# bytedance/particle-sfm

Measured on AMD Instinct MI355X. Metric: trajectory-points/s, higher is better.
Workload: dtype f32 sampling + f64 positions; 1 GPU; configs[1]: synthetic 100x(1920x1080) flow pairs, sample_ratio=2, flow_check + chaining + occlusion + id assignment, 1 sequence per GPU; frames=101, height=1080, width=1920, trajectories=2073277, parallelism=sequence-per-gpu x1, world_size=1

## Files before the change

### particle-sfm_amd/csrc/psfm_api.hip

```cpp
#include <stdarg.h>
#include <stdio.h>
#include <string.h>
#include <mutex>
#include <shared_mutex>
#include <atomic>
#include <chrono>
#include <stdlib.h>

#include "psfm_internal.h"

static thread_local char g_err[512] = "";
static std::shared_mutex g_dev_gate[16];
std::shared_mutex& psfm_device_gate(int device) { return g_dev_gate[device & 15]; }
static std::atomic<int> g_dev_waiters[16];
int psfm_gate_waiters(int device) { return g_dev_waiters[device & 15].load(std::memory_order_relaxed); }
void psfm_gate_waiters_add(int device, int d) { g_dev_waiters[device & 15].fetch_add(d, std::memory_order_relaxed); }
static int psfm_wants_persist(psfm_ctx* c, bool optimize, int h, int w, int ratio, bool fused)
{
    if (c->chain_mode == 1 || ratio < 1 || !psfm_frame_ok(h, w)) return 0;
    if (optimize) return c->resident_budget > 0 ? 0 : 1;
    const int64_t G = (int64_t)((w + ratio - 1) / ratio) * ((h + ratio - 1) / ratio);
    const int64_t P = (int64_t)h * w;
    const int maxb = psfm_persist_max_blocks(c);
    if (maxb <= 0 || (G + 255) / 256 > maxb) return 0;
// ... 81 lines not shown
void PsfmProfiler::reset()
{
    for (int k = 0; k < PSFM_PROF_KINDS; ++k) { total_ms[k] = 0; launches[k] = 0; }
}
void PsfmProfiler::destroy()
{
    collect();
    for (auto e : pool) (void)hipEventDestroy(e);
    pool.clear();
}

#define PSFM_CHECK_CTX(c)                                                     \
    do {                                                                      \
        if (!(c)) { psfm_set_error("ctx is NULL"); return PSFM_ERR_ARG; }     \
        PSFM_HIP(hipSetDevice((c)->device));                                  \
    } while (0)

extern "C" psfm_status psfm_ctx_create(int device, psfm_ctx** out)
{
    if (!out) { psfm_set_error("psfm_ctx_create: out is NULL"); return PSFM_ERR_ARG; }
    *out = nullptr;
    int n = 0;
    hipError_t e = hipGetDeviceCount(&n);
    if (e != hipSuccess || n <= 0) {
        (void)hipGetLastError();
        psfm_set_error("no HIP device available (%s); libpsfm_hip has no CPU fallback",
                       e != hipSuccess ? hipGetErrorString(e) : "device count 0");
        return PSFM_ERR_HIP;
    }
    if (device < 0 || device >= n) { psfm_set_error("device %d out of range [0,%d)", device, n); return PSFM_ERR_ARG; }
    PSFM_HIP(hipSetDevice(device));
    psfm_ctx* c = new psfm_ctx();
    c->device = device;
    c->host_pinned_bytes = 512 + sizeof(PsfmShard) * PSFM_NSHARD + 4096;
    e = hipHostMalloc(&c->host_pinned, c->host_pinned_bytes, hipHostMallocDefault);
    if (e != hipSuccess) { delete c; psfm_set_error("hipHostMalloc failed: %s", hipGetErrorString(e)); return PSFM_ERR_HIP; }
    *out = c;
    return PSFM_OK;
}

extern "C" psfm_status psfm_ctx_destroy(psfm_ctx* c)
{
    if (!c) return PSFM_OK;
    (void)hipSetDevice(c->device);
    PsfmBuf* bufs[] = {&c->log, &c->birth_frame, &c->birth_idx, &c->free_stack, &c->fin_keys, &c->fin_lanes,
                       &c->occupied, &c->counters, &c->shards, &c->survivors, &c->sort_keys, &c->sort_lanes, &c->sort_tmp,
                       &c->scan_tmp, &c->fin_marks, &c->res_birth, &c->res_len, &c->res_off, &c->res_xy, &c->sol_x, &c->sol_state,
                       &c->sol_partials, &c->sol_ctrl, &c->sol_misc, &c->sol_stats, &c->sol_fused, &c->sol_bar, &c->sol_list, &c->occ_own, &c->occ2_own,
                       &c->handoff, &c->seg_info, &c->seg_table, &c->persist_bar, &c->batch_tab, &c->batch_ws, &c->batch_fc, &c->win_ws, &c->flt_ids, &c->flt_birth, &c->flt_len, &c->flt_off, &c->flt_xy,
                       &c->mt_kp_off, &c->mt_q, &c->mt_pts, &c->mt_kp_ind, &c->mt_kp_xy, &c->mt_moff, &c->mt_keys, &c->mt_rows, &c->mt_gid, &c->mt_pairs,
                       &c->lb_state, &c->lb_first, &c->lb_flag, &c->lb_ws, &c->lb_ids, &c->lb_off, &c->lb_frames, &c->lb_xy, &c->lb_labels, &c->gt_flag};
    for (auto b : bufs) b->release();
    for (void*& q : c->peer_opened) { if (q) (void)hipIpcCloseMemHandle(q); q = nullptr; }
    c->peer_area.release();
    psfm_shard_abandon(c);
    c->prof.destroy();
    if (c->side_stream) (void)hipStreamDestroy(c->side_stream);
    if (c->redo_stream) (void)hipStreamDestroy(c->redo_stream);
    if (c->copy_stream) (void)hipStreamDestroy(c->copy_stream);
    if (c->copy_stream2) (void)hipStreamDestroy(c->copy_stream2);
    for (void* p : c->ingest_slots) (void)hipHostFree(p);
    for (hipEvent_t e : c->ingest_events) (void)hipEventDestroy(e);
    if (c->host_pinned) (void)hipHostFree(c->host_pinned);
    if (c->host_seg) (void)hipHostFree(c->host_seg);
    if (c->host_batch) (void)hipHostFree(c->host_batch);
    if (c->host_batch2) (void)hipHostFree(c->host_batch2);
    delete c;
    return PSFM_OK;
}
// ... 246 lines not shown
    psfm_status st;
    if ((st = psfm_track_dims(c, n_flows, h, w, ratio, -1, d)) != PSFM_OK) return st;
    const int64_t P = (int64_t)h * w;
    if ((st = psfm_track_alloc(c, d)) != PSFM_OK) return st;

    c->solve_stats.clear();
    c->res_n_traj = c->res_n_points = 0;
    c->res_n_flows = n_flows;
    c->pc_persist_ok = device_is_ours || c->resident_budget > 0;
    c->pc_giveups = 0;

    if (!optimize && c->chain_mode != 1) {
        const int maxb = psfm_persist_max_blocks(c);
        const int64_t need_blocks = (d.G + 255) / 256;
        if (maxb > 0 && need_blocks <= maxb && device_is_ours) {
            PsfmTrackDims dp = d;
            int64_t nb = need_blocks <= 256 ? 2 * need_blocks + 4 : need_blocks + need_blocks / 4;
            dp.nblk = (int)(nb < maxb ? nb : maxb);
            if (fuse_flows_b) {
                const int64_t fc_blocks = (P + 1023) / 1024;
                const int64_t want = fc_blocks < maxb ? fc_blocks : maxb;
                if (want > dp.nblk) dp.nblk = (int)want;
            }
            dp.cap = (int64_t)dp.nblk * (256 + psfm_persist_guests());
            dp.nsh = dp.nblk < PSFM_NSHARD ? dp.nblk : PSFM_NSHARD;
            dp.free_cap = (int)(((dp.nblk + dp.nsh - 1) / dp.nsh) * 256) + 1024;
            dp.seg_cap = (int)(d.traj_cap / dp.nblk) + 64;
            dp.spill_cap = (int)(d.traj_cap / 8) + 4096;
            const int64_t fin_total = (int64_t)dp.nblk * dp.seg_cap + dp.spill_cap;
            if ((st = c->log.ensure(sizeof(double2) * (size_t)(n_flows + 1) * dp.cap)) != PSFM_OK) return st;
            if ((st = c->free_stack.ensure(sizeof(int) * (size_t)dp.free_cap * PSFM_NSHARD * 2)) != PSFM_OK) return st;
            if ((st = c->fin_keys.ensure(sizeof(unsigned long long) * fin_total)) != PSFM_OK) return st;
            if ((st = c->fin_lanes.ensure(sizeof(int) * fin_total)) != PSFM_OK) return st;
            if ((st = c->handoff.ensure((size_t)dp.nblk * 256 * 24)) != PSFM_OK) return st;
            if ((st = c->seg_info.ensure(sizeof(int) * 2 * (size_t)dp.nblk)) != PSFM_OK) return st;
            if ((st = c->persist_bar.ensure((size_t)(4 * PSFM_NSHARD + 1) * 128)) != PSFM_OK) return st;
            if (pipe && (st = pipe->need(n_flows - 1, false, s)) != PSFM_OK) return st;
            bool fallback = false;
            {
                const bool trace = getenv("PSFM_TRACE") != nullptr;
                const auto t1 = std::chrono::steady_clock::now();
                st = psfm_launch_chain_persist(c, dp, flows, occ, occ_pitch, fuse_flows_b, fuse_thres, s);
                if (st == PSFM_ERR_CAPACITY) {
                    fallback = true;
                    st = PSFM_OK;
                } else {
                    if (st != PSFM_OK) return st;
                    c->prof.begin(PSFM_PROF_FINALIZE, s);
                    st = psfm_finalize_persist(c, dp, &fallback, s);
                    c->prof.end(s);
                }
                if (trace) {
                    const auto t2 = std::chrono::steady_clock::now();
                    fprintf(stderr, "[psfm %p] persistent loop: launch+finalize %.2f ms, fallback %d, overflow %d\n", (void*)c,
                            std::chrono::duration<double, std::milli>(t2 - t1).count(), (int)fallback,
                            ((PsfmCounters*)c->host_pinned)->overflow);
                }
            }
            if (st != PSFM_OK) return st;
            if (!fallback) {
                PSFM_HIP(hipStreamSynchronize(s));
                c->prof.collect();
                if (info) {
                    memset(info, 0, sizeof(*info));
                    info->n_traj = c->res_n_traj;
                    info->n_points = c->res_n_points;
                    info->n_lanes_peak = ((PsfmCounters*)c->host_pinned)->n_lanes;
                    info->lane_capacity = dp.cap;
                    info->chain_mode = 2;
                }
                return PSFM_OK;
            }
            c->prof.collect();
        }
    }
    if (fuse_flows_b) {
        c->prof.begin(PSFM_PROF_FLOW_CHECK, s);
        for (int f = 0; f < n_flows; ++f)
            if ((st = psfm_launch_flow_check(flows + (size_t)f * P * 2, fuse_flows_b + (size_t)f * P * 2, 1, h, w, fuse_thres,
                                             const_cast<uint8_t*>(occ) + (size_t)f * occ_pitch, nullptr, s)) != PSFM_OK) return st;
        c->prof.end(s);
    }
    if ((st = psfm_launch_track_init(c, d, s)) != PSFM_OK) return st;
    int64_t total_iters = 0;
    static const int check_env = getenv("PSFM_CHECK_FRAMES") ? atoi(getenv("PSFM_CHECK_FRAMES")) : 0;
    const int PSFM_CHECK = check_env >= 2 ? check_env : 16;
    std::vector<psfm_solve_stats> hstats((size_t)n_flows + 1);
    int first_unchecked = 1;
    if (optimize) {
// ... 308 lines not shown
```

### particle-sfm_amd/csrc/psfm_finalize.hip

```cpp
#include <cstring>
#include <stdio.h>
#include <rocprim/device/device_radix_sort.hpp>
#include <rocprim/device/device_scan.hpp>

#include "psfm_device.h"
#include "psfm_internal.h"

#define PSFM_BLOCK 256

__device__ __forceinline__ void psfm_collect_alive_body(
    const int* __restrict__ birth_frame, const int* __restrict__ birth_idx, PsfmCounters* __restrict__ ctr,
    PsfmShard* __restrict__ shards, unsigned long long* __restrict__ fin_keys, int* __restrict__ fin_lanes, int cap,
    int shard_cap, int last_time, int shift_b, int shift_d)
{
    __shared__ int s_cnt[PSFM_BLOCK / PSFM_WAVE];
    __shared__ int s_base;
    const int n_lanes = min(ctr->n_lanes, cap);
    if ((int)(blockIdx.x * PSFM_BLOCK) >= n_lanes) return;
    const int i = blockIdx.x * PSFM_BLOCK + threadIdx.x;
    int bf = -1;
    if (i < n_lanes) bf = birth_frame[i];
    const bool pending = bf <= -2;
    const bool alive = (bf >= 0) | pending;
    const int my_last = pending ? last_time - 1 : last_time;
// ... 380 lines not shown
#pragma unroll
            for (int k = 0; k < TILE_K; ++k) {
                const int t = k0 + k;
                if (t >= 1 && t < l) { pos.x = pos.x + (double)f[k].x; pos.y = pos.y + (double)f[k].y; }
                tile[tid][k] = pos;
            }
            s_pos[tid] = pos;
        }
        __syncthreads();
        const int kk = tid & (TILE_K - 1);
        for (int jj = tid / TILE_K; jj < TILE_J; jj += PSFM_BLOCK / TILE_K) {
            const int t = k0 + kk;
            if (t < s_len[jj]) out[s_off[jj] + t] = tile[jj][kk];
        }
        __syncthreads();
    }
}

static PsfmKeyFmt psfm_key_fmt(const PsfmTrackDims& d, unsigned* end_bit)
{
    PsfmKeyFmt f;
    f.shift_b = d.shift_b; f.shift_d = d.shift_d;
    const long long lmax = (long long)d.n_flows + 1;
    const long long tri_max = lmax * (lmax + 1) / 2 + lmax;
    int tri_bits = 1;
    while ((1ll << tri_bits) <= tri_max) ++tri_bits;
    f.use32 = (tri_bits + d.shift_b <= 32) ? 1 : 0;
    int tbits = 1;
    while ((1ll << tbits) < (long long)d.n_flows + 2) ++tbits;
    *end_bit = f.use32 ? (unsigned)(tri_bits + d.shift_b) : (unsigned)(d.shift_d + tbits);
    return f;
}

static bool psfm_own_sort(const PsfmKeyFmt& fmt, int64_t n)
{
    static const int on = getenv("PSFM_FIN_SORT") ? atoi(getenv("PSFM_FIN_SORT")) : 1;
    return on && fmt.use32 && n < (1ll << 31);
}
static bool psfm_records_in_first_half(const PsfmTrackDims& d, int64_t n)
{
    unsigned end_bit = 0;
    const PsfmKeyFmt fmt = psfm_key_fmt(d, &end_bit);
    return psfm_own_sort(fmt, n) && (psfm_sort_pairs32_passes(end_bit) % 2 == 0);
}

static psfm_status psfm_finalize_sorted(psfm_ctx* c, const PsfmTrackDims& d, int64_t n, int64_t npts, bool delta_log, hipStream_t s)
{
    psfm_status st;
    unsigned end_bit = 0;
    const PsfmKeyFmt fmt = psfm_key_fmt(d, &end_bit);
    int* l_in = c->sort_lanes.as<int>() + n;
    int* l_out = c->sort_lanes.as<int>();
    size_t tmp_bytes = 0, scan_bytes = 0;
    PSFM_HIP(rocprim::exclusive_scan(nullptr, scan_bytes, (int64_t*)nullptr, (int64_t*)nullptr, (int64_t)0,
                                     (size_t)(n + 1), rocprim::plus<int64_t>(), s));
    if (psfm_own_sort(fmt, n)) {
        if ((st = c->sort_tmp.ensure(scan_bytes)) != PSFM_OK) return st;
        if ((st = psfm_sort_pairs32(c, c->sort_keys.as<unsigned>(), l_out, c->sort_keys.as<unsigned>() + n, l_in, n, end_bit, s)) != PSFM_OK) return st;
    } else if (fmt.use32) {
        unsigned* k_in = c->sort_keys.as<unsigned>() + n;
        unsigned* k_out = c->sort_keys.as<unsigned>();
        PSFM_HIP(rocprim::radix_sort_pairs(nullptr, tmp_bytes, k_in, k_out, l_in, l_out, (size_t)n, 0u, end_bit, s));
        if ((st = c->sort_tmp.ensure(tmp_bytes > scan_bytes ? tmp_bytes : scan_bytes)) != PSFM_OK) return st;
        PSFM_HIP(rocprim::radix_sort_pairs(c->sort_tmp.p, tmp_bytes, k_in, k_out, l_in, l_out, (size_t)n, 0u, end_bit, s));
    } else {
        unsigned long long* k_in = c->sort_keys.as<unsigned long long>() + n;
        unsigned long long* k_out = c->sort_keys.as<unsigned long long>();
        PSFM_HIP(rocprim::radix_sort_pairs(nullptr, tmp_bytes, k_in, k_out, l_in, l_out, (size_t)n, 0u, end_bit, s));
        if ((st = c->sort_tmp.ensure(tmp_bytes > scan_bytes ? tmp_bytes : scan_bytes)) != PSFM_OK) return st;
        PSFM_HIP(rocprim::radix_sort_pairs(c->sort_tmp.p, tmp_bytes, k_in, k_out, l_in, l_out, (size_t)n, 0u, end_bit, s));
    }
    if ((st = c->res_birth.ensure(sizeof(int) * n)) != PSFM_OK) return st;
    if ((st = c->res_len.ensure(sizeof(int) * n)) != PSFM_OK) return st;
    if ((st = c->res_off.ensure(sizeof(int64_t) * (n + 1))) != PSFM_OK) return st;
    static const int plan_on = getenv("PSFM_FIN_PLAN") ? atoi(getenv("PSFM_FIN_PLAN")) : 1;
    const long long lmax = (long long)d.n_flows + 1;
    const long long ng = lmax * (lmax + 1) / 2 + lmax + 1;
    PsfmPlan pl;
    pl.gstart = nullptr; pl.goff = nullptr; pl.keys = (const void*)c->sort_keys.p; pl.use32 = fmt.use32; pl.shift_b = d.shift_b; pl.shift_d = d.shift_d;
    pl.birth_w = c->res_birth.as<int>(); pl.len_w = c->res_len.as<int>(); pl.off_w = c->res_off.as<int64_t>();
    if (plan_on && ng <= PSFM_PLAN_MAX_GROUPS && n < (1ll << 31)) {
        if ((st = c->scan_tmp.ensure((sizeof(int64_t) + sizeof(int)) * (size_t)ng)) != PSFM_OK) return st;
        int64_t* goff = c->scan_tmp.as<int64_t>();
        int* gstart = (int*)(goff + ng);
        const void* had = c->fin_marks.p;
        if ((st = c->fin_marks.ensure(sizeof(int) * (size_t)PSFM_PLAN_MAX_GROUPS)) != PSFM_OK) return st;
        if (!c->fin_marks_clean || had != c->fin_marks.p)
            PSFM_HIP(hipMemsetAsync(c->fin_marks.p, 0xff, sizeof(int) * (size_t)PSFM_PLAN_MAX_GROUPS, s));
        c->fin_marks_clean = false;
        hipLaunchKernelGGL(psfm_group_bounds_kernel, dim3((unsigned)((n + PSFM_BLOCK - 1) / PSFM_BLOCK)), dim3(PSFM_BLOCK), 0, s,
                           (const void*)c->sort_keys.p, n, fmt.use32, d.shift_b, d.shift_d, c->fin_marks.as<int>());
        hipLaunchKernelGGL(psfm_group_plan_kernel, dim3(1), dim3(PSFM_PLAN_BLOCK), 0, s, c->fin_marks.as<int>(), gstart, goff, (int)ng, n,
                           c->res_off.as<int64_t>() + n);
        PSFM_HIP(hipGetLastError());
        c->fin_marks_clean = true;
        pl.gstart = gstart; pl.goff = goff;
    } else {
        if ((st = c->scan_tmp.ensure(sizeof(int64_t) * (n + 1))) != PSFM_OK) return st;
        if (fmt.use32)
// ... 37 lines not shown
    PSFM_HIP(hipMemcpyAsync(hc, ctr, sizeof(PsfmCounters), hipMemcpyDeviceToHost, s));
    PSFM_HIP(hipMemcpyAsync(hs, shards, sizeof(PsfmShard) * PSFM_NSHARD, hipMemcpyDeviceToHost, s));
    PSFM_HIP(hipStreamSynchronize(s));
    PsfmShardOffsets so;
    int64_t n = 0, npts = 0;
    bool over = hc->overflow != 0;
    for (int k = 0; k < PSFM_NSHARD; ++k) npts += hs[k].points;
    for (int k = 0; k < PSFM_NSHARD; ++k) {
        if (hs[k].fin_cnt > d.shard_cap) over = true;
        so.count[k] = hs[k].fin_cnt > d.shard_cap ? d.shard_cap : hs[k].fin_cnt;
        so.start[k] = n;
        n += so.count[k];
    }
    if (over || hc->n_lanes > d.cap) {
        psfm_set_error("capacity exceeded: lanes used %d of %lld, trajectory records %lld of %lld (%d shards); "
                       "raise psfm_ctx_set_capacity", hc->n_lanes, (long long)d.cap, (long long)n,
                       (long long)d.traj_cap, PSFM_NSHARD);
        return PSFM_ERR_CAPACITY;
    }
    c->res_n_traj = n;
    c->res_n_points = 0;
    if (n == 0) return PSFM_OK;
    psfm_status st;
    if ((st = c->sort_keys.ensure(sizeof(unsigned long long) * n * 2)) != PSFM_OK) return st;
    if ((st = c->sort_lanes.ensure(sizeof(int) * n * 2)) != PSFM_OK) return st;
    unsigned end_bit_unused = 0;
    const PsfmKeyFmt fmt = psfm_key_fmt(d, &end_bit_unused);
    const int64_t half = psfm_records_in_first_half(d, n) ? 0 : n;
    unsigned long long* kdst = fmt.use32 ? (unsigned long long*)(c->sort_keys.as<unsigned>() + half) : c->sort_keys.as<unsigned long long>() + half;
    hipLaunchKernelGGL(psfm_compact_shards_kernel, dim3(64, PSFM_NSHARD), dim3(PSFM_BLOCK), 0, s,
                       c->fin_keys.as<unsigned long long>(), c->fin_lanes.as<int>(), d.shard_cap, so,
                       kdst, c->sort_lanes.as<int>() + half, fmt);
    PSFM_HIP(hipGetLastError());
    return psfm_finalize_sorted(c, d, n, npts, false, s);
}

__global__ __launch_bounds__(PSFM_BLOCK) void psfm_compact_segments_kernel(
    const unsigned long long* __restrict__ fin_keys, const int* __restrict__ fin_lanes, const int2* __restrict__ seg_info, int nblk,
    int seg_cap, const PsfmCounters* __restrict__ ctr, int spill_cap, unsigned long long* __restrict__ keys, int* __restrict__ lanes,
    PsfmKeyFmt fmt)
{
    __shared__ long long s_part[PSFM_BLOCK / PSFM_WAVE];
    const int b = blockIdx.x, tid = threadIdx.x;
    long long mine = 0;
    for (int k = tid; k < b; k += PSFM_BLOCK) mine += seg_info[k].x;
#pragma unroll
    for (int o = 32; o > 0; o >>= 1) mine += __shfl_down(mine, o);
    if ((tid & (PSFM_WAVE - 1)) == 0) s_part[tid / PSFM_WAVE] = mine;
    __syncthreads();
    long long dst = 0;
    for (int w = 0; w < PSFM_BLOCK / PSFM_WAVE; ++w) dst += s_part[w];
    const int count = b < nblk ? seg_info[b].x : min(ctr->spill_cnt, spill_cap);
    const long long src = (long long)b * seg_cap;
    for (int i0 = 0; i0 < count; i0 += 4 * PSFM_BLOCK) {
        unsigned long long k[4];
        int l[4];
#pragma unroll
        for (int u = 0; u < 4; ++u) {
            const int i = i0 + u * PSFM_BLOCK + tid;
            k[u] = i < count ? fin_keys[src + i] : 0ull;
            l[u] = i < count ? fin_lanes[src + i] : 0;
        }
#pragma unroll
        for (int u = 0; u < 4; ++u) {
            const int i = i0 + u * PSFM_BLOCK + tid;
            if (i < count) {
                psfm_put_key(keys, dst + i, k[u], fmt);
                lanes[dst + i] = l[u];
            }
        }
    }
}

psfm_status psfm_finalize_persist(psfm_ctx* c, const PsfmTrackDims& d, bool* fallback, hipStream_t s)
{
    *fallback = false;
    const int nseg = d.nblk + 1;
    const size_t need = sizeof(int2) * (size_t)d.nblk;
    if (c->host_seg_bytes < need) {
        if (c->host_seg) (void)hipHostFree(c->host_seg);
        c->host_seg = nullptr; c->host_seg_bytes = 0;
        PSFM_HIP(hipHostMalloc(&c->host_seg, need, hipHostMallocDefault));
        c->host_seg_bytes = need;
    }
    int2* hinfo = (int2*)c->host_seg;
    PsfmCounters* hc = (PsfmCounters*)c->host_pinned;
    PSFM_HIP(hipMemcpyAsync(hc, c->counters.p, sizeof(PsfmCounters), hipMemcpyDeviceToHost, s));
    PSFM_HIP(hipMemcpyAsync(hinfo, c->seg_info.p, sizeof(int2) * (size_t)d.nblk, hipMemcpyDeviceToHost, s));
    PSFM_HIP(hipStreamSynchronize(s));
    if (hc->pad[0]) fprintf(stderr, "psfm persist check: site %d index %d\n", hc->pad[0], hc->pad[1]);
    if (hc->overflow & (4 | 8)) {
        *fallback = true;
        return PSFM_OK;
    }
    int64_t n = 0, npts = 0;
    for (int b = 0; b < d.nblk; ++b) {
        n += hinfo[b].x;
        npts += hinfo[b].y;
    }
    const int spilled = hc->spill_cnt < d.spill_cap ? hc->spill_cnt : d.spill_cap;
    n += spilled;
    if (hc->overflow != 0) {
        psfm_set_error("capacity exceeded (persistent loop): overflow bits %d, trajectory records %lld (%d spilled of %d); "
                       "raise psfm_ctx_set_capacity", hc->overflow, (long long)n, hc->spill_cnt, d.spill_cap);
        return PSFM_ERR_CAPACITY;
    }
    c->res_n_traj = n;
    c->res_n_points = 0;
    if (n == 0) return PSFM_OK;
    psfm_status st;
    if ((st = c->sort_keys.ensure(sizeof(unsigned long long) * n * 2)) != PSFM_OK) return st;
    if ((st = c->sort_lanes.ensure(sizeof(int) * n * 2)) != PSFM_OK) return st;
    unsigned end_bit_unused = 0;
    const PsfmKeyFmt fmt = psfm_key_fmt(d, &end_bit_unused);
    const int64_t half = psfm_records_in_first_half(d, n) ? 0 : n;
    unsigned long long* kdst = fmt.use32 ? (unsigned long long*)(c->sort_keys.as<unsigned>() + half) : c->sort_keys.as<unsigned long long>() + half;
    hipLaunchKernelGGL(psfm_compact_segments_kernel, dim3((unsigned)nseg), dim3(PSFM_BLOCK), 0, s,
                       c->fin_keys.as<unsigned long long>(), c->fin_lanes.as<int>(), (const int2*)c->seg_info.as<int2>(), d.nblk, d.seg_cap,
                       (const PsfmCounters*)c->counters.as<PsfmCounters>(), d.spill_cap, kdst, c->sort_lanes.as<int>() + half, fmt);
    PSFM_HIP(hipGetLastError());
    return psfm_finalize_sorted(c, d, n, npts, true, s);
}

struct PsfmFinSeq {
    const int* birth_frame; const int* birth_idx; PsfmCounters* ctr; PsfmShard* shards;
    unsigned long long* fin_keys; int* fin_lanes;
    const double2* log; int64_t cap;
    int shard_cap, last_time;
    int64_t rec_start, n;
    int* res_birth; int* res_len; int64_t* res_off; double2* res_xy;
};

__global__ __launch_bounds__(PSFM_BLOCK) void psfm_collect_alive_batch_kernel(const PsfmFinSeq* __restrict__ T, int shift_b, int shift_d)
{
    const PsfmFinSeq& q = T[blockIdx.y];
    psfm_collect_alive_body(q.birth_frame, q.birth_idx, q.ctr, q.shards, q.fin_keys, q.fin_lanes, (int)q.cap, q.shard_cap, q.last_time,
                            shift_b, shift_d);
}

__global__ __launch_bounds__(PSFM_WAVE) void psfm_batch_counts_kernel(const PsfmFinSeq* __restrict__ T, long long* __restrict__ counts)
{
    const PsfmFinSeq& q = T[blockIdx.x];
    const int k = threadIdx.x;
    static_assert(PSFM_NSHARD == PSFM_WAVE, "one lane per shard");
    const int fc = q.shards[k].fin_cnt;
    long long n = fc > q.shard_cap ? q.shard_cap : fc;
    long long pts = q.shards[k].points;
    int over = fc > q.shard_cap ? 1 : 0;
#pragma unroll
    for (int o = 32; o > 0; o >>= 1) { n += __shfl_down(n, o); pts += __shfl_down(pts, o); over |= __shfl_down(over, o); }
    if (k == 0) {
        counts[blockIdx.x * 4 + 0] = n;
        counts[blockIdx.x * 4 + 1] = pts;
        counts[blockIdx.x * 4 + 2] = (long long)(q.ctr->overflow | (over ? 2 : 0));
// ... 194 lines not shown
```

### particle-sfm_amd/csrc/psfm_internal.h

```cpp
#pragma once
#include <hip/hip_runtime.h>
#include <stdint.h>
#include <shared_mutex>
#include <string>
#include <vector>

#include "../../include/psfm.h"

#define PSFM_MAX_PEERS 8

void psfm_set_error(const char* fmt, ...);

#define PSFM_HIP(expr)                                                                          \
    do {                                                                                        \
        hipError_t e_ = (expr);                                                                 \
        if (e_ != hipSuccess) {                                                                 \
            psfm_set_error("%s failed: %s (%s:%d)", #expr, hipGetErrorString(e_), __FILE__, __LINE__); \
            return PSFM_ERR_HIP;                                                                \
        }                                                                                       \
    } while (0)

static inline bool psfm_frame_ok(int h, int w) { return h >= 2 && w >= 2 && (int64_t)h * (int64_t)w * 8 < ((int64_t)1 << 32); }

std::shared_mutex& psfm_device_gate(int device);
int psfm_gate_waiters(int device);
void psfm_gate_waiters_add(int device, int d);
struct PsfmGate {
    std::shared_mutex& m;
    int device;
    bool exclusive = false;
    PsfmGate(int dev, int want_exclusive ) : m(psfm_device_gate(dev)), device(dev)
    {
        if (want_exclusive == 2) { m.lock(); exclusive = true; }
        else if (want_exclusive == 1 && m.try_lock()) exclusive = true;
        else if (!m.try_lock_shared()) {
            psfm_gate_waiters_add(device, 1);
            m.lock_shared();
            psfm_gate_waiters_add(device, -1);
        }
    }
// ... 115 lines not shown
    PsfmBuf occ_own, occ2_own;
    PsfmBuf batch_tab, batch_ws, batch_fc;
    void* host_batch = nullptr;
    size_t host_batch_bytes = 0;
    void* host_batch2 = nullptr;
    size_t host_batch2_bytes = 0;
    int64_t batch_notrim_shape = 0;
    PsfmBuf win_ws;
    PsfmBuf flt_ids, flt_birth, flt_len, flt_off, flt_xy;
    int64_t flt_n_traj = 0, flt_n_points = 0;
    PsfmBuf mt_kp_off, mt_q, mt_pts, mt_kp_ind, mt_kp_xy, mt_moff, mt_keys, mt_rows, mt_gid, mt_pairs;
    int64_t mt_n_kp = 0, mt_n_m = 0, mt_n_pairs = 0;
    int mt_n_img = 0;
    uint64_t res_gen = 0;
    uint64_t lb_gen = 0;
    bool lb_active = false, lb_finished = false;
    int64_t lb_rows = 0;
    PsfmBuf lb_state, lb_first, lb_flag;
    PsfmBuf lb_ws;
    PsfmBuf lb_ids, lb_off, lb_frames, lb_xy, lb_labels;
    int64_t lb_n_traj = 0, lb_n_points = 0;
    PsfmBuf gt_flag;
    hipStream_t side_stream = nullptr;
    hipStream_t copy_stream = nullptr;
    hipStream_t copy_stream2 = nullptr;
    std::vector<void*> ingest_slots;
    std::vector<hipEvent_t> ingest_events;
    size_t ingest_slot_bytes = 0;
    hipStream_t redo_stream = nullptr;
    std::vector<psfm_solve_stats> solve_stats;
    PsfmProfiler prof;
    void* host_pinned = nullptr;
    size_t host_pinned_bytes = 0;
};

psfm_status psfm_launch_flow_check(const float* ff, const float* fb, int n_pairs, int h, int w, float thres,
                                   uint8_t* occ, float* err, hipStream_t s);
psfm_status psfm_launch_flow_check_bg(const float* ff, const float* fb, int n_pairs, int h, int w, float thres, uint8_t* occ,
                                      int n_blocks, hipStream_t s);
psfm_status psfm_launch_grid_sample(const float* map, int c, int h, int w, const double* xy, int64_t n,
                                    float* out, hipStream_t s);

struct PsfmTrackDims {
    int H, W, ratio, GW, GH, n_flows;
    int64_t G, cap, traj_cap;
    int shard_cap;
    int free_cap;
    int nsh = PSFM_NSHARD;
    int shift_b, shift_d;
    float cw, ch;
    int nblk = 0, seg_cap = 0, spill_cap = 0;
    int64_t g0 = 0, Gband = 0, shard_pitch = 0;
    uint8_t* shard_maps = nullptr;
};

psfm_status psfm_track_dims(psfm_ctx* c, int n_flows, int h, int w, int ratio, int64_t g_own, PsfmTrackDims& d);
psfm_status psfm_track_alloc(psfm_ctx* c, const PsfmTrackDims& d);
psfm_status psfm_launch_track_init(psfm_ctx* c, const PsfmTrackDims& d, hipStream_t s);
psfm_status psfm_launch_chain_step(psfm_ctx* c, const PsfmTrackDims& d, const float* flow, const uint8_t* occ,
                                   int frame, bool optimize, hipStream_t s);

#define PSFM_BATCH_MAX 64
struct PsfmBatchSeq;
struct PsfmFcSeq { const float* ff; const float* fb; uint8_t* occ; int n_pairs; int pad; };
bool psfm_flow_check_batch_ok(int h, int w, const void* ff, const void* fb, const void* occ);
psfm_status psfm_launch_flow_check_batch(const PsfmFcSeq* tab_dev, int n_seq, int pair0, int n_pairs, int h, int w, float thres, hipStream_t s);
// ... 69 lines not shown
```

### particle-sfm_amd/csrc/psfm_persist.hip

```cpp
#include <hip/hip_ext.h>
#include <stdlib.h>

#include "psfm_internal.h"
#include "psfm_chain.h"

#define PP_BLOCK 256
#define PP_NW (PP_BLOCK / PSFM_WAVE)
#define PP_PROBE 8
#ifndef PP_PRE_WAVES
#define PP_PRE_WAVES 4
#endif
#ifndef PP_KEEP
#define PP_KEEP 0
#endif
#ifndef PP_FC_AHEAD
#define PP_FC_AHEAD 4
#endif
#ifndef PP_FC_PAIRS
#define PP_FC_PAIRS 1
#endif
#define PP_GUESTS 32
#ifndef PP_WHATIF
#define PP_WHATIF 0
#endif
// ... 641 lines not shown
    const int lane = tid & (PSFM_WAVE - 1), wave = tid / PSFM_WAVE;
    {
        const int nf = PA->n_flows;
        const bool alive = bf >= 0;
        const int slot = psfm_record_slot(&s_rec_cnt, alive);
        if (alive) psfm_put_record(slot, psfm_cold_key(nf, bf, s_gi[tid]), L);
        if (tid < PP_GUESTS && s_gbf[tid] >= 0) {
            const int gslot = atomicAdd(&s_rec_cnt, 1);
            psfm_put_record(gslot, psfm_cold_key(nf, s_gbf[tid], s_ggi[tid]),
                            psfm_cold()->cap_main + PP_BID * PP_GUESTS + tid);
        }
    }
    {
        __shared__ int s_pts[PP_NW];
        int w = s_npts[tid];
#pragma unroll
        for (int o = 32; o > 0; o >>= 1) w += __shfl_down(w, o);
        if (lane == 0) s_pts[wave] = w;
        __syncthreads();
        if (tid == 0) {
            int tot = 0;
            for (int j = 0; j < PP_NW; ++j) tot += s_pts[j];
            const int c = s_rec_cnt;
            const PsfmColdPtr cold = psfm_cold();
            const int seg_cap = cold->seg_cap;
            cold->seg_info[PP_BID] = make_int2(c < seg_cap ? c : seg_cap, tot);
        }
    }
}

__global__ __launch_bounds__(256) void psfm_persist_init_kernel(PsfmCounters* ctr, PsfmShard* shards, int G,
                                                                unsigned long long* maps64, size_t n_maps64,
                                                                unsigned long long* bar64, size_t n_bar64,
                                                                unsigned long long* handoff, size_t n_handoff)
{
    const size_t i = (size_t)blockIdx.x * 256 + threadIdx.x, stride = (size_t)gridDim.x * 256;
    if (i == 0) { ctr->n_lanes = G; ctr->overflow = 0; ctr->stall = 0; ctr->abort = 0; ctr->spill_cnt = 0; ctr->pad[0] = 0; ctr->pad[1] = 0; }
    if (i < 2 * PSFM_NSHARD) { shards[i].fin_cnt = 0; shards[i].free_top = 0; shards[i].points = 0u; }
    for (size_t k = i; k < n_maps64; k += stride) maps64[k] = 0ull;
    for (size_t k = i; k < n_bar64; k += stride) bar64[k] = 0ull;
    for (size_t k = i; k < n_handoff; k += stride) handoff[k] = ~0ull;
}

int psfm_persist_guests(void) { return PP_GUESTS; }

int psfm_persist_max_blocks(psfm_ctx* c)
{
    if (c->persist_max_blocks >= 0) return c->persist_max_blocks;
    int cus = 0;
    c->persist_max_blocks = 0;
    if (hipDeviceGetAttribute(&cus, hipDeviceAttributeMultiprocessorCount, c->device) != hipSuccess) {
        (void)hipGetLastError();
        return 0;
    }
    int per_cu = 1 << 30;
    const void* inst[4] = {(const void*)psfm_chain_persist_kernel<0>, (const void*)psfm_chain_persist_kernel<1>,
                           (const void*)psfm_chain_persist_kernel<2>, (const void*)psfm_chain_persist_kernel<4>};
    for (int k = 0; k < 4; ++k) {
        int v = 0;
        if (hipOccupancyMaxActiveBlocksPerMultiprocessor(&v, inst[k], PP_BLOCK, 0) != hipSuccess) {
            (void)hipGetLastError();
            return 0;
        }
        per_cu = v < per_cu ? v : per_cu;
    }
    if (per_cu > 8) per_cu = 8;
    c->persist_max_blocks = per_cu * cus;
    return c->persist_max_blocks;
}

psfm_status psfm_launch_chain_persist(psfm_ctx* c, const PsfmTrackDims& d, const float* flows, const uint8_t* occ,
                                      int64_t occ_pitch, const float* flows_b, float thres, hipStream_t s)
{
    const size_t bar_bytes = (size_t)(4 * PSFM_NSHARD + 1) * 128;
    {
        const size_t n_maps64 = ((size_t)d.G * 3 + 7) / 8, n_bar64 = bar_bytes / 8, n_handoff = (size_t)d.nblk * PP_BLOCK * 3;
        hipLaunchKernelGGL(psfm_persist_init_kernel, dim3(1024), dim3(256), 0, s, c->counters.as<PsfmCounters>(),
                           c->shards.as<PsfmShard>(), (int)d.G, c->occupied.as<unsigned long long>(), n_maps64,
                           c->persist_bar.as<unsigned long long>(), n_bar64, c->handoff.as<unsigned long long>(), n_handoff);
    }
    PsfmPersistKernarg ka;
    PsfmPersistArgs& a = ka.hot;
    PsfmPersistCold& k = ka.cold;
    a.flows = (const float2*)flows; a.occ = const_cast<uint8_t*>(occ);
    a.occ_pitch = occ_pitch;
    a.flows_b = (const float2*)flows_b; a.t2 = psfm_sq_threshold(thres); a.fc = flows_b != nullptr;
    {
        static const int xcd_on = getenv("PSFM_FC_XCD") ? atoi(getenv("PSFM_FC_XCD")) : 1;
        const int64_t nch = ((int64_t)d.H * d.W + 1023) / 1024;
        a.fc_xcd_per = xcd_on && nch >= 64 ? (int)((nch + 7) / 8) : 0;
    }
    {
        static const int pp_xcd = getenv("PSFM_PP_XCD") ? atoi(getenv("PSFM_PP_XCD")) : 1;
        const int64_t gb = (d.G + PP_BLOCK - 1) / PP_BLOCK;
        const int per = (int)((gb + 7) / 8);
        a.xcd_per = (pp_xcd && gb >= 64 && 8 * per <= d.nblk) ? per : 0;
    }
    a.wdiv = psfm_fastdiv_make((unsigned)d.W);
    a.H = d.H; a.W = d.W; a.cw = d.cw; a.ch = d.ch; a.rcw = psfm_rcp_host(d.cw); a.rch = psfm_rcp_host(d.ch);
    a.ratio = d.ratio; a.GW = d.GW; a.GH = d.GH; a.G = (int)d.G;
    a.dlog = c->log.as<float2>(); a.cap = k.cap = (int)d.cap; k.cap_main = d.nblk * PP_BLOCK;
    a.maps = c->occupied.as<uint8_t>();
    k.ctr = c->counters.as<PsfmCounters>();
    k.shards = c->shards.as<PsfmShard>();
    k.free_stack = c->free_stack.as<int>(); k.free_cap = d.free_cap; k.nsh = d.nsh;
    a.handoff = c->handoff.as<unsigned long long>();
    k.fin_keys = c->fin_keys.as<unsigned long long>(); k.fin_lanes = c->fin_lanes.as<int>();
    k.seg_cap = d.seg_cap; k.spill_base = d.nblk * d.seg_cap; k.spill_cap = d.spill_cap;
    k.seg_info = c->seg_info.as<int2>();
    a.bar = c->persist_bar.as<unsigned>();
    a.n_flows = d.n_flows; a.nblk = d.nblk; k.shift_b = d.shift_b; k.shift_d = d.shift_d;
    a.gwdiv = psfm_fastdiv_make((unsigned)d.GW); a.rdiv = psfm_fastdiv_make((unsigned)d.ratio);
// ... 30 lines not shown
```

Measured before the change: 22.27 billion trajectory-points/s.

## Publish finalize totals via mapped host memory and launch compaction before readback

The compaction kernel is now launched immediately after the persistent loop. It is sized for worst-case capacity, and an extra block reduces the segment counts and writes the totals plus counters into coherent, mapped pinned host memory, guarded by a sequence number. The host spin-polls that record instead of doing two device-to-host copies and a full stream synchronize before launching compaction. This removes a sync round trip from the finalize path. In exchange it allocates sort buffers at full capacity, adds CPU busy-waiting, and zeroes seg_info in the init kernel.

```diff
diff --git a/particle-sfm_amd/csrc/psfm_api.hip b/particle-sfm_amd/csrc/psfm_api.hip
--- a/particle-sfm_amd/csrc/psfm_api.hip
+++ b/particle-sfm_amd/csrc/psfm_api.hip
@@ -137,9 +137,21 @@
     PSFM_HIP(hipSetDevice(device));
     psfm_ctx* c = new psfm_ctx();
     c->device = device;
-    c->host_pinned_bytes = 512 + sizeof(PsfmShard) * PSFM_NSHARD + 4096;
-    e = hipHostMalloc(&c->host_pinned, c->host_pinned_bytes, hipHostMallocDefault);
+    const size_t pub_off = 512 + sizeof(PsfmShard) * PSFM_NSHARD + 4096;
+    c->host_pinned_bytes = pub_off;
+    e = hipHostMalloc(&c->host_pinned, pub_off + sizeof(PsfmPublish), hipHostMallocCoherent | hipHostMallocMapped);
     if (e != hipSuccess) { delete c; psfm_set_error("hipHostMalloc failed: %s", hipGetErrorString(e)); return PSFM_ERR_HIP; }
+    memset(c->host_pinned, 0, pub_off + sizeof(PsfmPublish));
+    c->pub = (PsfmPublish*)((char*)c->host_pinned + pub_off);
+    void* pub_dev = nullptr;
+    e = hipHostGetDevicePointer(&pub_dev, c->pub, 0);
+    if (e != hipSuccess) {
+        (void)hipHostFree(c->host_pinned);
+        delete c;
+        psfm_set_error("hipHostGetDevicePointer failed: %s", hipGetErrorString(e));
+        return PSFM_ERR_HIP;
+    }
+    c->pub_dev = (PsfmPublish*)pub_dev;
     *out = c;
     return PSFM_OK;
 }
@@ -452,6 +464,8 @@
             if ((st = c->free_stack.ensure(sizeof(int) * (size_t)dp.free_cap * PSFM_NSHARD * 2)) != PSFM_OK) return st;
             if ((st = c->fin_keys.ensure(sizeof(unsigned long long) * fin_total)) != PSFM_OK) return st;
             if ((st = c->fin_lanes.ensure(sizeof(int) * fin_total)) != PSFM_OK) return st;
+            if ((st = c->sort_keys.ensure(sizeof(unsigned long long) * fin_total * 2)) != PSFM_OK) return st;
+            if ((st = c->sort_lanes.ensure(sizeof(int) * fin_total * 2)) != PSFM_OK) return st;
             if ((st = c->handoff.ensure((size_t)dp.nblk * 256 * 24)) != PSFM_OK) return st;
             if ((st = c->seg_info.ensure(sizeof(int) * 2 * (size_t)dp.nblk)) != PSFM_OK) return st;
             if ((st = c->persist_bar.ensure((size_t)(4 * PSFM_NSHARD + 1) * 128)) != PSFM_OK) return st;
@@ -472,9 +486,9 @@
                 }
                 if (trace) {
                     const auto t2 = std::chrono::steady_clock::now();
-                    fprintf(stderr, "[psfm %p] persistent loop: launch+finalize %.2f ms, fallback %d, overflow %d\n", (void*)c,
+                    fprintf(stderr, "[psfm %p] persistent loop: launch+finalize %.2f ms, fallback %d, overflow %d, spilled %d of %d\n", (void*)c,
                             std::chrono::duration<double, std::milli>(t2 - t1).count(), (int)fallback,
-                            ((PsfmCounters*)c->host_pinned)->overflow);
+                            ((PsfmCounters*)c->host_pinned)->overflow, ((PsfmCounters*)c->host_pinned)->spill_cnt, dp.spill_cap);
                 }
             }
             if (st != PSFM_OK) return st;
diff --git a/particle-sfm_amd/csrc/psfm_finalize.hip b/particle-sfm_amd/csrc/psfm_finalize.hip
--- a/particle-sfm_amd/csrc/psfm_finalize.hip
+++ b/particle-sfm_amd/csrc/psfm_finalize.hip
@@ -436,39 +436,40 @@
     return f;
 }
 
-static bool psfm_own_sort(const PsfmKeyFmt& fmt, int64_t n)
+static bool psfm_own_sort(const PsfmKeyFmt& fmt, int64_t half_stride)
 {
     static const int on = getenv("PSFM_FIN_SORT") ? atoi(getenv("PSFM_FIN_SORT")) : 1;
-    return on && fmt.use32 && n < (1ll << 31);
-}
-static bool psfm_records_in_first_half(const PsfmTrackDims& d, int64_t n)
+    return on && fmt.use32 && half_stride < (1ll << 31);
+}
+static bool psfm_records_in_first_half(const PsfmTrackDims& d, int64_t half_stride)
 {
     unsigned end_bit = 0;
     const PsfmKeyFmt fmt = psfm_key_fmt(d, &end_bit);
-    return psfm_own_sort(fmt, n) && (psfm_sort_pairs32_passes(end_bit) % 2 == 0);
-}
-
-static psfm_status psfm_finalize_sorted(psfm_ctx* c, const PsfmTrackDims& d, int64_t n, int64_t npts, bool delta_log, hipStream_t s)
+    return psfm_own_sort(fmt, half_stride) && (psfm_sort_pairs32_passes(end_bit) % 2 == 0);
+}
+
+static psfm_status psfm_finalize_sorted(psfm_ctx* c, const PsfmTrackDims& d, int64_t n, int64_t npts, bool delta_log, int64_t half_stride,
+                                        hipStream_t s)
 {
     psfm_status st;
     unsigned end_bit = 0;
     const PsfmKeyFmt fmt = psfm_key_fmt(d, &end_bit);
-    int* l_in = c->sort_lanes.as<int>() + n;
+    int* l_in = c->sort_lanes.as<int>() + half_stride;
     int* l_out = c->sort_lanes.as<int>();
     size_t tmp_bytes = 0, scan_bytes = 0;
     PSFM_HIP(rocprim::exclusive_scan(nullptr, scan_bytes, (int64_t*)nullptr, (int64_t*)nullptr, (int64_t)0,
                                      (size_t)(n + 1), rocprim::plus<int64_t>(), s));
-    if (psfm_own_sort(fmt, n)) {
+    if (psfm_own_sort(fmt, half_stride)) {
         if ((st = c->sort_tmp.ensure(scan_bytes)) != PSFM_OK) return st;
-        if ((st = psfm_sort_pairs32(c, c->sort_keys.as<unsigned>(), l_out, c->sort_keys.as<unsigned>() + n, l_in, n, end_bit, s)) != PSFM_OK) return st;
+        if ((st = psfm_sort_pairs32(c, c->sort_keys.as<unsigned>(), l_out, c->sort_keys.as<unsigned>() + half_stride, l_in, n, end_bit, s)) != PSFM_OK) return st;
     } else if (fmt.use32) {
-        unsigned* k_in = c->sort_keys.as<unsigned>() + n;
+        unsigned* k_in = c->sort_keys.as<unsigned>() + half_stride;
         unsigned* k_out = c->sort_keys.as<unsigned>();
         PSFM_HIP(rocprim::radix_sort_pairs(nullptr, tmp_bytes, k_in, k_out, l_in, l_out, (size_t)n, 0u, end_bit, s));
         if ((st = c->sort_tmp.ensure(tmp_bytes > scan_bytes ? tmp_bytes : scan_bytes)) != PSFM_OK) return st;
         PSFM_HIP(rocprim::radix_sort_pairs(c->sort_tmp.p, tmp_bytes, k_in, k_out, l_in, l_out, (size_t)n, 0u, end_bit, s));
     } else {
-        unsigned long long* k_in = c->sort_keys.as<unsigned long long>() + n;
+        unsigned long long* k_in = c->sort_keys.as<unsigned long long>() + half_stride;
         unsigned long long* k_out = c->sort_keys.as<unsigned long long>();
         PSFM_HIP(rocprim::radix_sort_pairs(nullptr, tmp_bytes, k_in, k_out, l_in, l_out, (size_t)n, 0u, end_bit, s));
         if ((st = c->sort_tmp.ensure(tmp_bytes > scan_bytes ? tmp_bytes : scan_bytes)) != PSFM_OK) return st;
@@ -572,25 +573,57 @@
                        c->fin_keys.as<unsigned long long>(), c->fin_lanes.as<int>(), d.shard_cap, so,
                        kdst, c->sort_lanes.as<int>() + half, fmt);
     PSFM_HIP(hipGetLastError());
-    return psfm_finalize_sorted(c, d, n, npts, false, s);
-}
-
+    return psfm_finalize_sorted(c, d, n, npts, false, n, s);
+}
+
+__device__ __forceinline__ int psfm_seg_count(const int2* __restrict__ seg_info, int k, int seg_cap)
+{
+    return min(max(seg_info[k].x, 0), seg_cap);
+}
 __global__ __launch_bounds__(PSFM_BLOCK) void psfm_compact_segments_kernel(
     const unsigned long long* __restrict__ fin_keys, const int* __restrict__ fin_lanes, const int2* __restrict__ seg_info, int nblk,
     int seg_cap, const PsfmCounters* __restrict__ ctr, int spill_cap, unsigned long long* __restrict__ keys, int* __restrict__ lanes,
-    PsfmKeyFmt fmt)
-{
-    __shared__ long long s_part[PSFM_BLOCK / PSFM_WAVE];
-    const int b = blockIdx.x, tid = threadIdx.x;
+    PsfmKeyFmt fmt, PsfmPublish* __restrict__ pub, unsigned long long seq)
+{
+    __shared__ long long s_part[2][PSFM_BLOCK / PSFM_WAVE];
+    const int tid = threadIdx.x;
+    if (blockIdx.x == 0) {
+        long long recs = 0, pts = 0;
+        for (int k = tid; k < nblk; k += PSFM_BLOCK) {
+            recs += psfm_seg_count(seg_info, k, seg_cap);
+            pts += seg_info[k].y;
+        }
+#pragma unroll
+        for (int o = 32; o > 0; o >>= 1) { recs += __shfl_down(recs, o); pts += __shfl_down(pts, o); }
+        if ((tid & (PSFM_WAVE - 1)) == 0) { s_part[0][tid / PSFM_WAVE] = recs; s_part[1][tid / PSFM_WAVE] = pts; }
+        __syncthreads();
+        if (tid == 0) {
+            recs = 0; pts = 0;
+            for (int w = 0; w < PSFM_BLOCK / PSFM_WAVE; ++w) { recs += s_part[0][w]; pts += s_part[1][w]; }
+            const int spill = ctr->spill_cnt;
+            recs += min(max(spill, 0), spill_cap);
+            __hip_atomic_store(&pub->n, recs, __ATOMIC_RELAXED, __HIP_MEMORY_SCOPE_SYSTEM);
+            __hip_atomic_store(&pub->npts, pts, __ATOMIC_RELAXED, __HIP_MEMORY_SCOPE_SYSTEM);
+            __hip_atomic_store(&pub->overflow, ctr->overflow, __ATOMIC_RELAXED, __HIP_MEMORY_SCOPE_SYSTEM);
+            __hip_atomic_store(&pub->spill_cnt, spill, __ATOMIC_RELAXED, __HIP_MEMORY_SCOPE_SYSTEM);
+            __hip_atomic_store(&pub->n_lanes, ctr->n_lanes, __ATOMIC_RELAXED, __HIP_MEMORY_SCOPE_SYSTEM);
+            __hip_atomic_store(&pub->pad[0], ctr->pad[0], __ATOMIC_RELAXED, __HIP_MEMORY_SCOPE_SYSTEM);
+            __hip_atomic_store(&pub->pad[1], ctr->pad[1], __ATOMIC_RELAXED, __HIP_MEMORY_SCOPE_SYSTEM);
+            __builtin_amdgcn_fence(__ATOMIC_RELEASE, "");
+            __hip_atomic_store(&pub->seq, seq, __ATOMIC_RELAXED, __HIP_MEMORY_SCOPE_SYSTEM);
+        }
+        return;
+    }
+    const int b = (int)blockIdx.x - 1;
     long long mine = 0;
-    for (int k = tid; k < b; k += PSFM_BLOCK) mine += seg_info[k].x;
+    for (int k = tid; k < b; k += PSFM_BLOCK) mine += psfm_seg_count(seg_info, k, seg_cap);
 #pragma unroll
     for (int o = 32; o > 0; o >>= 1) mine += __shfl_down(mine, o);
-    if ((tid & (PSFM_WAVE - 1)) == 0) s_part[tid / PSFM_WAVE] = mine;
+    if ((tid & (PSFM_WAVE - 1)) == 0) s_part[0][tid / PSFM_WAVE] = mine;
     __syncthreads();
     long long dst = 0;
-    for (int w = 0; w < PSFM_BLOCK / PSFM_WAVE; ++w) dst += s_part[w];
-    const int count = b < nblk ? seg_info[b].x : min(ctr->spill_cnt, spill_cap);
+    for (int w = 0; w < PSFM_BLOCK / PSFM_WAVE; ++w) dst += s_part[0][w];
+    const int count = b < nblk ? psfm_seg_count(seg_info, b, seg_cap) : min(max(ctr->spill_cnt, 0), spill_cap);
     const long long src = (long long)b * seg_cap;
     for (int i0 = 0; i0 < count; i0 += 4 * PSFM_BLOCK) {
         unsigned long long k[4];
@@ -612,54 +645,63 @@
     }
 }
 
+static int psfm_publish_query(void* stream)
+{
+    const hipError_t e = hipStreamQuery((hipStream_t)stream);
+    if (e == hipSuccess) return PSFM_PUBQ_DONE;
+    if (e == hipErrorNotReady) { (void)hipGetLastError(); return PSFM_PUBQ_BUSY; }
+    return 2 + (int)e;
+}
+
 psfm_status psfm_finalize_persist(psfm_ctx* c, const PsfmTrackDims& d, bool* fallback, hipStream_t s)
 {
     *fallback = false;
     const int nseg = d.nblk + 1;
-    const size_t need = sizeof(int2) * (size_t)d.nblk;
-    if (c->host_seg_bytes < need) {
-        if (c->host_seg) (void)hipHostFree(c->host_seg);
-        c->host_seg = nullptr; c->host_seg_bytes = 0;
-        PSFM_HIP(hipHostMalloc(&c->host_seg, need, hipHostMallocDefault));
-        c->host_seg_bytes = need;
-    }
-    int2* hinfo = (int2*)c->host_seg;
+    const int64_t fin_total = (int64_t)d.nblk * d.seg_cap + d.spill_cap;
+    psfm_status st;
+    if ((st = c->sort_keys.ensure(sizeof(unsigned long long) * fin_total * 2)) != PSFM_OK) return st;
+    if ((st = c->sort_lanes.ensure(sizeof(int) * fin_total * 2)) != PSFM_OK) return st;
+    unsigned end_bit_unused = 0;
+    const PsfmKeyFmt fmt = psfm_key_fmt(d, &end_bit_unused);
+    const int64_t half = psfm_records_in_first_half(d, fin_total) ? 0 : fin_total;
+    unsigned long long* kdst = fmt.use32 ? (unsigned long long*)(c->sort_keys.as<unsigned>() + half) : c->sort_keys.as<unsigned long long>() + half;
+    const unsigned long long seq = ++c->pub_seq;
+    hipLaunchKernelGGL(psfm_compact_segments_kernel, dim3((unsigned)nseg + 1u), dim3(PSFM_BLOCK), 0, s,
+                       c->fin_keys.as<unsigned long long>(), c->fin_lanes.as<int>(), (const int2*)c->seg_info.as<int2>(), d.nblk, d.seg_cap,
+                       (const PsfmCounters*)c->counters.as<PsfmCounters>(), d.spill_cap, kdst, c->sort_lanes.as<int>() + half, fmt,
+                       c->pub_dev, seq);
+    PSFM_HIP(hipGetLastError());
+    PsfmPublish rec;
+    int qerr = 0;
+    const int w = psfm_publish_wait(c->pub, seq, psfm_publish_query, (void*)s, &rec, &qerr);
+    if (w == PSFM_PUB_QUERY) {
+        const hipError_t e = (hipError_t)(qerr - 2);
+        (void)hipGetLastError();
+        psfm_set_error("hipStreamQuery failed while waiting for the finalize's totals: %s (%s:%d)", hipGetErrorString(e), __FILE__, __LINE__);
+        return PSFM_ERR_HIP;
+    }
+    if (w != PSFM_PUB_OK) {
+        psfm_set_error("internal error: the stream completed without the finalize's totals of call %llu (record says %llu)", seq,
+                       (unsigned long long)c->pub->seq);
+        return PSFM_ERR_HIP;
+    }
     PsfmCounters* hc = (PsfmCounters*)c->host_pinned;
-    PSFM_HIP(hipMemcpyAsync(hc, c->counters.p, sizeof(PsfmCounters), hipMemcpyDeviceToHost, s));
-    PSFM_HIP(hipMemcpyAsync(hinfo, c->seg_info.p, sizeof(int2) * (size_t)d.nblk, hipMemcpyDeviceToHost, s));
-    PSFM_HIP(hipStreamSynchronize(s));
-    if (hc->pad[0]) fprintf(stderr, "psfm persist check: site %d index %d\n", hc->pad[0], hc->pad[1]);
-    if (hc->overflow & (4 | 8)) {
+    hc->n_lanes = rec.n_lanes; hc->overflow = rec.overflow; hc->spill_cnt = rec.spill_cnt; hc->pad[0] = rec.pad[0]; hc->pad[1] = rec.pad[1];
+    if (rec.pad[0]) fprintf(stderr, "psfm persist check: site %d index %d\n", rec.pad[0], rec.pad[1]);
+    if (rec.overflow & (4 | 8)) {
         *fallback = true;
         return PSFM_OK;
     }
-    int64_t n = 0, npts = 0;
-    for (int b = 0; b < d.nblk; ++b) {
-        n += hinfo[b].x;
-        npts += hinfo[b].y;
-    }
-    const int spilled = hc->spill_cnt < d.spill_cap ? hc->spill_cnt : d.spill_cap;
-    n += spilled;
-    if (hc->overflow != 0) {
+    const int64_t n = rec.n, npts = rec.npts;
+    if (rec.overflow != 0) {
         psfm_set_error("capacity exceeded (persistent loop): overflow bits %d, trajectory records %lld (%d spilled of %d); "
-                       "raise psfm_ctx_set_capacity", hc->overflow, (long long)n, hc->spill_cnt, d.spill_cap);
+                       "raise psfm_ctx_set_capacity", rec.overflow, (long long)n, rec.spill_cnt, d.spill_cap);
         return PSFM_ERR_CAPACITY;
     }
     c->res_n_traj = n;
     c->res_n_points = 0;
     if (n == 0) return PSFM_OK;
-    psfm_status st;
-    if ((st = c->sort_keys.ensure(sizeof(unsigned long long) * n * 2)) != PSFM_OK) return st;
-    if ((st = c->sort_lanes.ensure(sizeof(int) * n * 2)) != PSFM_OK) return st;
-    unsigned end_bit_unused = 0;
-    const PsfmKeyFmt fmt = psfm_key_fmt(d, &end_bit_unused);
-    const int64_t half = psfm_records_in_first_half(d, n) ? 0 : n;
-    unsigned long long* kdst = fmt.use32 ? (unsigned long long*)(c->sort_keys.as<unsigned>() + half) : c->sort_keys.as<unsigned long long>() + half;
-    hipLaunchKernelGGL(psfm_compact_segments_kernel, dim3((unsigned)nseg), dim3(PSFM_BLOCK), 0, s,
-                       c->fin_keys.as<unsigned long long>(), c->fin_lanes.as<int>(), (const int2*)c->seg_info.as<int2>(), d.nblk, d.seg_cap,
-                       (const PsfmCounters*)c->counters.as<PsfmCounters>(), d.spill_cap, kdst, c->sort_lanes.as<int>() + half, fmt);
-    PSFM_HIP(hipGetLastError());
-    return psfm_finalize_sorted(c, d, n, npts, true, s);
+    return psfm_finalize_sorted(c, d, n, npts, true, fin_total, s);
 }
 
 struct PsfmFinSeq {
diff --git a/particle-sfm_amd/csrc/psfm_internal.h b/particle-sfm_amd/csrc/psfm_internal.h
--- a/particle-sfm_amd/csrc/psfm_internal.h
+++ b/particle-sfm_amd/csrc/psfm_internal.h
@@ -6,6 +6,7 @@
 #include <vector>
 
 #include "../../include/psfm.h"
+#include "psfm_publish.h"
 
 #define PSFM_MAX_PEERS 8
 
@@ -187,6 +188,9 @@
     PsfmProfiler prof;
     void* host_pinned = nullptr;
     size_t host_pinned_bytes = 0;
+    PsfmPublish* pub = nullptr;
+    PsfmPublish* pub_dev = nullptr;
+    unsigned long long pub_seq = 0;
 };
 
 psfm_status psfm_launch_flow_check(const float* ff, const float* fb, int n_pairs, int h, int w, float thres,
diff --git a/particle-sfm_amd/csrc/psfm_persist.hip b/particle-sfm_amd/csrc/psfm_persist.hip
--- a/particle-sfm_amd/csrc/psfm_persist.hip
+++ b/particle-sfm_amd/csrc/psfm_persist.hip
@@ -697,9 +697,11 @@
 __global__ __launch_bounds__(256) void psfm_persist_init_kernel(PsfmCounters* ctr, PsfmShard* shards, int G,
                                                                 unsigned long long* maps64, size_t n_maps64,
                                                                 unsigned long long* bar64, size_t n_bar64,
-                                                                unsigned long long* handoff, size_t n_handoff)
+                                                                unsigned long long* handoff, size_t n_handoff,
+                                                                unsigned long long* seg_info64, size_t n_seg)
 {
     const size_t i = (size_t)blockIdx.x * 256 + threadIdx.x, stride = (size_t)gridDim.x * 256;
+    for (size_t k = i; k < n_seg; k += stride) seg_info64[k] = 0ull;
     if (i == 0) { ctr->n_lanes = G; ctr->overflow = 0; ctr->stall = 0; ctr->abort = 0; ctr->spill_cnt = 0; ctr->pad[0] = 0; ctr->pad[1] = 0; }
     if (i < 2 * PSFM_NSHARD) { shards[i].fin_cnt = 0; shards[i].free_top = 0; shards[i].points = 0u; }
     for (size_t k = i; k < n_maps64; k += stride) maps64[k] = 0ull;
@@ -742,7 +744,8 @@
         const size_t n_maps64 = ((size_t)d.G * 3 + 7) / 8, n_bar64 = bar_bytes / 8, n_handoff = (size_t)d.nblk * PP_BLOCK * 3;
         hipLaunchKernelGGL(psfm_persist_init_kernel, dim3(1024), dim3(256), 0, s, c->counters.as<PsfmCounters>(),
                            c->shards.as<PsfmShard>(), (int)d.G, c->occupied.as<unsigned long long>(), n_maps64,
-                           c->persist_bar.as<unsigned long long>(), n_bar64, c->handoff.as<unsigned long long>(), n_handoff);
+                           c->persist_bar.as<unsigned long long>(), n_bar64, c->handoff.as<unsigned long long>(), n_handoff,
+                           c->seg_info.as<unsigned long long>(), (size_t)d.nblk);
     }
     PsfmPersistKernarg ka;
     PsfmPersistArgs& a = ka.hot;
diff --git a/particle-sfm_amd/csrc/psfm_publish.h b/particle-sfm_amd/csrc/psfm_publish.h
--- /dev/null
+++ b/particle-sfm_amd/csrc/psfm_publish.h
@@ -0,0 +1,68 @@
+#pragma once
+#include <stdint.h>
+
+struct PsfmPublish {
+    long long n;
+    long long npts;
+    int overflow, spill_cnt, n_lanes;
+    int pad[2];
+    int reserved[5];
+    unsigned long long seq;
+};
+static_assert(sizeof(PsfmPublish) == 64, "one line");
+
+#ifndef PSFM_PUBLISH_POLLS
+#define PSFM_PUBLISH_POLLS 4096
+#endif
+static inline void psfm_publish_relax(void)
+{
+#if defined(__x86_64__) || defined(__i386__)
+    __builtin_ia32_pause();
+#endif
+}
+
+enum { PSFM_PUBQ_DONE = 0, PSFM_PUBQ_BUSY = 1 };
+enum { PSFM_PUB_OK = 0,
+       PSFM_PUB_STALE = 1,
+       PSFM_PUB_QUERY = 2 };
+
+static inline bool psfm_publish_take(const volatile PsfmPublish* rec, unsigned long long expect, PsfmPublish* out)
+{
+    if (__atomic_load_n(&rec->seq, __ATOMIC_ACQUIRE) != expect) return false;
+    out->n = rec->n; out->npts = rec->npts;
+    out->overflow = rec->overflow; out->spill_cnt = rec->spill_cnt; out->n_lanes = rec->n_lanes;
+    out->pad[0] = rec->pad[0]; out->pad[1] = rec->pad[1];
+    out->seq = expect;
+    return true;
+}
+
+static inline int psfm_publish_wait(const volatile PsfmPublish* rec, unsigned long long expect, int (*query)(void*), void* user,
+                                    PsfmPublish* out, int* query_err, unsigned long long* polls = nullptr,
+                                    unsigned long long* queries = nullptr)
+{
+    unsigned long long np = 0, nq = 0;
+    int rc;
+    for (;;) {
+        bool got = false;
+        for (int k = 0; k < PSFM_PUBLISH_POLLS && !got; ++k) {
+            ++np;
+            got = psfm_publish_take(rec, expect, out);
+            if (!got) psfm_publish_relax();
+        }
+        if (got) { rc = PSFM_PUB_OK; break; }
+        ++nq;
+        const int q = query(user);
+        if (q == PSFM_PUBQ_BUSY) continue;
+        if (q == PSFM_PUBQ_DONE) {
+            ++np;
+            rc = psfm_publish_take(rec, expect, out) ? PSFM_PUB_OK : PSFM_PUB_STALE;
+            break;
+        }
+        if (query_err) *query_err = q;
+        rc = PSFM_PUB_QUERY;
+        break;
+    }
+    if (polls) *polls = np;
+    if (queries) *queries = nq;
+    return rc;
+}
```

Measured after the change: 22.37 billion trajectory-points/s, median of 6. About the same (+0.4%).
